# APRIL-ZJU/Ctrl-VIO

Hardware: NVIDIA H100
Metric: residual+Jacobian block evaluations per second (sliding-window LM solve) (higher is better)
Workload: dtype f64

## Files before the change

### ctrl-vio_b200/csrc/chol_dag.cu

```cuda
#include <algorithm>
#include <atomic>
#include <cstdlib>

#include "chol_tiles.cuh"
#include "dmma_tiles.cuh"
#include "kernels.h"

namespace ctvio {

namespace {

__device__ __forceinline__ int ld_acquire(const int* p) {
  int v;
  asm volatile("ld.acquire.gpu.global.s32 %0, [%1];" : "=r"(v) : "l"(p) : "memory");
  return v;
}
__device__ __forceinline__ void st_release(int* p, int v) {
  asm volatile("st.release.gpu.global.s32 [%0], %1;" ::"l"(p), "r"(v) : "memory");
}
constexpr unsigned long long kSentinel = 0xFFF8C0DEC0DE0001ull;
__device__ __forceinline__ unsigned smem_u32(const void* p) { return static_cast<unsigned>(__cvta_generic_to_shared(p)); }
__device__ __forceinline__ unsigned mapa_u32(unsigned addr, unsigned rank) {
  unsigned r;
  asm volatile("mapa.shared::cluster.u32 %0, %1, %2;" : "=r"(r) : "r"(addr), "r"(rank));
  return r;
}
__device__ __forceinline__ void st_cluster2(unsigned addr, double2 v) {
  asm volatile("st.shared::cluster.v2.f64 [%0], {%1, %2};" ::"r"(addr), "d"(v.x), "d"(v.y) : "memory");
}
__device__ __forceinline__ double2 ld_shared_volatile2(const double* p) {
  double2 v;
  asm volatile("ld.volatile.shared.v2.f64 {%0, %1}, [%2];" : "=d"(v.x), "=d"(v.y) : "r"(smem_u32(p)) : "memory");
  return v;
}
__device__ __forceinline__ void cluster_arrive() { asm volatile("barrier.cluster.arrive.release.aligned;" ::: "memory"); }
__device__ __forceinline__ void cluster_wait() { asm volatile("barrier.cluster.wait.acquire.aligned;" ::: "memory"); }
__device__ __forceinline__ unsigned cluster_ctarank() {
  unsigned r;
  asm volatile("mov.u32 %0, %%cluster_ctarank;" : "=r"(r));
  return r;
}
__device__ __forceinline__ unsigned cluster_nctarank() {
// ... 8 lines not shown
  return v;
}
__device__ __forceinline__ void st_relaxed2(double* p, double2 v) {
  asm volatile("st.relaxed.gpu.global.v2.f64 [%0], {%1, %2};" ::"l"(p), "d"(v.x), "d"(v.y) : "memory");
}

__device__ __forceinline__ double ld_relaxed1(const double* p) {
  double v;
  asm volatile("ld.relaxed.gpu.global.f64 %0, [%1];" : "=d"(v) : "l"(p) : "memory");
  return v;
}
__device__ __forceinline__ void st_relaxed1(double* p, double v) {
  asm volatile("st.relaxed.gpu.global.f64 [%0], %1;" ::"l"(p), "d"(v) : "memory");
}
__device__ __forceinline__ double ld_spin(const double* p) {
  double v = ld_relaxed1(p);
  while (is_sentinel(v)) v = ld_relaxed1(p);
  return v;
}
__device__ __forceinline__ double sentinel_value() { return __longlong_as_double(static_cast<long long>(kSentinel)); }

__device__ __forceinline__ void wait_flag(const int* flag, int epoch) {
  if (threadIdx.x == 0) {
    while (ld_acquire(flag) != epoch) {}
  }
  __syncthreads();
}
__device__ __forceinline__ void wait_flags2(const int* f1, const int* f2, int epoch) {
  if (threadIdx.x == 0) {
    while (ld_acquire(f1) != epoch) {}
  } else if (threadIdx.x == 32) {
    while (ld_acquire(f2) != epoch) {}
  }
  __syncthreads();
}
__device__ __forceinline__ void post_flag(int* flag, int epoch) {
  __syncthreads();
  if (threadIdx.x == 0) {
    __threadfence();
    st_release(flag, epoch);
  }
}

__device__ __forceinline__ void load_tile_cg(double* dst, const double* src, int ld, int tid) {
#pragma unroll
  for (int e = tid; e < kCholNB * kCholNB / 2; e += 256) {
    const int r = e >> 5, c = (e & 31) * 2;
    *reinterpret_cast<double2*>(dst + r * kTS + c) = __ldcg(reinterpret_cast<const double2*>(src + size_t(r) * ld + c));
  }
}
__device__ __forceinline__ void store_tile_global(double* dst, int ld, const double* src, int tid) {
#pragma unroll
  for (int e = tid; e < kCholNB * kCholNB / 2; e += 256) {
    const int r = e >> 5, c = (e & 31) * 2;
    *reinterpret_cast<double2*>(dst + size_t(r) * ld + c) = *reinterpret_cast<const double2*>(src + r * kTS + c);
  }
}
__device__ __forceinline__ double sum_partials(const double* part, int n, size_t stride, double* red, int tid) {
  const int c = tid & 63, g = tid >> 6;
  double s = 0.0;
  int q = g;
  for (; q + 12 < n; q += 16) {
    double v0 = ld_relaxed1(part + size_t(q) * stride + c), v1 = ld_relaxed1(part + size_t(q + 4) * stride + c);
// ... 609 lines not shown
```

### ctrl-vio_b200/csrc/engine.cu

```cuda
#include <atomic>
#include <cmath>
#include <cstdlib>
#include <map>

#include "engine_state.h"

namespace ctvio::host {

int refresh_mirror(ctvio_engine* e) {
  const size_t need = 4 * size_t(e->nK) + kPStride * size_t(e->nK) + 6 * size_t(std::max(e->nB, 1)) + size_t(std::max(e->nL, 1)) + 8;
  if (need > e->h_mirror_cap) {
    if (e->h_mirror) cudaFreeHost(e->h_mirror);
    e->h_mirror = nullptr;
    e->h_mirror_cap = 0;
    if (cudaHostAlloc(reinterpret_cast<void**>(&e->h_mirror), (2 * need) * sizeof(double), cudaHostAllocDefault) != cudaSuccess) {
      cudaGetLastError();
      e->mirror_valid = false;
      return CTVIO_OK;
    }
    e->h_mirror_cap = 2 * need;
  }
  DevState& x = e->x[e->cur];
  double* m = e->h_mirror;
  cudaStream_t st = e->stream;
// ... 258 lines not shown
        for (int x = 0; x < nbk; ++x)
          for (int y = 0; y <= x; ++y) {
            lists[size_t(blocks[x]) * (blocks[x] + 1) / 2 + blocks[y]].push_back(l);
            ++total;
          }
      }
      const int n_sm = device_sm_count();
      const int part = std::max(32, int((total / size_t(2 * n_sm) + 31) / 32) * 32);
      std::vector<SchurTileItem> items;
      std::vector<SchurEntry> flat;
      flat.reserve(total);
      for (int ti = 0; ti < T; ++ti)
        for (int tj = 0; tj <= ti; ++tj) {
          const std::vector<int32_t>& v = lists[size_t(ti) * (ti + 1) / 2 + tj];
          for (size_t s0 = 0; s0 < v.size(); s0 += part)
            items.push_back(SchurTileItem{ti, tj, int32_t(flat.size() + s0), int32_t(std::min(v.size() - s0, size_t(part)))});
          for (int32_t l : v) flat.push_back(SchurEntry{l, e->h_lo[l], e->h_hi[l], 0, e->h_woff[l]});
        }
      e->n_schur_items = int(items.size());
      e->n_schur_entries = int(flat.size());
      CUDA_OK(e->d_schur_list.upload(flat, st));
      CUDA_OK(e->d_schur_items.upload(items, st));
    }
    CUDA_OK(e->d_lis.reserve(e->nL));
    CUDA_OK(e->d_lc.reserve(e->nL));
    if (chol_dag_flags_len(e->npad) > e->d_chol_flags.cap) {
      CUDA_OK(e->d_chol_flags.reserve(chol_dag_flags_len(e->npad)));
      CUDA_OK(cudaMemsetAsync(e->d_chol_flags.p, 0, e->d_chol_flags.cap * sizeof(int32_t), e->stream));
    }
    CUDA_OK(e->d_y.reserve(e->npad));
    CUDA_OK(e->d_sc.reserve(np));
    CUDA_OK(e->d_sl.reserve(e->nL));
    CUDA_OK(e->d_hh.reserve(e->nL));
    CUDA_OK(e->d_dc.reserve(np));
    CUDA_OK(e->d_dl.reserve(e->nL));
    if (e->nL > 0) CUDA_OK(cudaMemsetAsync(e->d_hh.p, 0, sizeof(double) * e->nL, st));
    e->prior_dirty = true;
  }
  if (e->structure_dirty || e->masks_dirty) {
    e->h_cmask.assign(d.np, 0);
    for (int k = 0; k < e->nK; ++k)
      if (e->opt.lock_traj || (e->opt.fixed_knot_index >= 0 && k <= e->opt.fixed_knot_index))
        for (int c = 0; c < 6; ++c) e->h_cmask[6 * k + c] = 1;
    for (int b = 0; b < e->nB; ++b)
      for (int c = 0; c < 3; ++c) {
        if (e->opt.lock_wb) e->h_cmask[d.idx_bias0 + 6 * b + c] = 1;
        if (e->opt.lock_ab) e->h_cmask[d.idx_bias0 + 6 * b + 3 + c] = 1;
      }
// ... 146 lines not shown
  v.det_ticket = e->deterministic ? e->d_ticket.p : nullptr;
  return v;
}
SmallFactorsLaunch small_launch(ctvio_engine* e, int xb, int nb) {
  SmallFactorsLaunch v;
  v.bf = BiasFactorPtrs{e->d_bf_ij.p, e->d_bf_s.p, int32_t(e->biasf.size())};
  v.prior = prior_ptrs(e);
  v.st = e->state(xb).ptrs();
  v.ne = e->ne(nb);
  v.dims = e->dims();
  v.cmask = e->d_cmask.p;
  v.scal = e->d_scal.p;
  v.deterministic = e->deterministic ? 1 : 0;
  return v;
}
LinearLaunch linear_launch(ctvio_engine* e, int nb) {
  LinearLaunch a;
  a.dims = e->dims();
  a.ne = e->ne(nb);
  a.lm = e->lml();
  a.schur_list = e->d_schur_list.p;
  a.schur_items = e->d_schur_items.p;
  a.n_schur_items = e->n_schur_items;
  a.lis = e->d_lis.p; a.lc = e->d_lc.p;
  a.cmask = e->d_cmask.p;
  a.active = e->d_active.p;
  a.sc = e->d_sc.p; a.sl = e->d_sl.p;
  a.M = e->d_M.p; a.Linv = e->d_Linv.p; a.y = e->d_y.p;
  a.rhs = e->d_M.p + size_t(e->npad) * e->npad;
  a.diagA = a.rhs + e->npad;
  a.yf = a.diagA + e->npad;
  a.chol_part = e->d_chol_part.p; a.chol_flags = e->d_chol_flags.p; a.chol_seq = &e->chol_seq;
  a.sharded = e->world > 1 ? 1 : 0;
  a.hh = e->d_hh.p; a.dc = e->d_dc.p; a.dl = e->d_dl.p;
  a.npad = e->npad;
  a.scal = e->d_scal.p;
  a.go = nullptr;
  a.det_ticket = e->deterministic ? e->d_ticket.p : nullptr;
  return a;
}

void evaluate(ctvio_engine* e, int xb, int nb, bool full, bool reset_cost) {
  cudaStream_t st = e->stream;
  if (full) {
    if (e->slab_zeroed[nb]) {
      cudaStreamWaitEvent(st, e->ev_zero, 0);
      e->slab_zeroed[nb] = false;
// ... 687 lines not shown
  for (int r = 0; r < reps; ++r) {
    if (r > 0) CUDA_OK(cudaMemcpyAsync(lin.M, backup.p, len * sizeof(double), cudaMemcpyDeviceToDevice, st));
    launch_factor_solve(lin, st);
    CUDA_OK(cudaMemcpyAsync((r == 0 ? x0 : x).data(), lin.y, n * sizeof(double), cudaMemcpyDeviceToHost, st));
    CUDA_OK(cudaStreamSynchronize(st));
    if (r > 0 && std::memcmp(x.data(), x0.data(), n * sizeof(double)) != 0) ++*mismatches;
  }
  for (size_t i = 0; i < n; ++i)
    for (size_t j = i + 1; j < n; ++j) hM[i * n + j] = hM[j * n + i];
  const double* rhs = hM.data() + n * n;
  double rmax = 0, bmax = 0;
  for (size_t i = 0; i < n; ++i) {
    double s = -rhs[i];
    for (size_t j = 0; j < n; ++j) s += hM[i * n + j] * x0[j];
    rmax = std::max(rmax, std::fabs(s));
    bmax = std::max(bmax, std::fabs(rhs[i]));
  }
  *rel_residual = bmax > 0 ? rmax / bmax : rmax;
  cudaMemsetAsync(&e->d_scal.p->error_flags, 0, sizeof(int32_t), st);
  CUDA_OK(cudaStreamSynchronize(st));
  return CTVIO_OK;
}

int ctvio_debug_lm_step(ctvio_handle e, double radius, double* out, int64_t* len) {
  if (!e || !len || !(radius > 0.0)) return fail(CTVIO_ERR_INVALID, "bad argument");
  cudaSetDevice(e->cfg.device);
  int rc = prepare(e);
  if (rc) return rc;
  const ProblemDims d = e->dims();
  const size_t np = size_t(d.np), nL = size_t(e->nL), npad = size_t(e->npad);
  const size_t need = 16 + np * np + np + 2 * nL + nL * np + 2 * np + 2 * nL + npad * npad + 2 * npad + np + nL;
  const int64_t cap = *len;
  *len = int64_t(need);
  if (!out) return CTVIO_OK;
  if (cap < int64_t(need)) return fail(CTVIO_ERR_INVALID, "output slab too small");
  ensure_table(e);
  cudaStream_t st = e->stream;
  const int cur = e->cur;
  evaluate(e, cur, cur, true);
  rc = read_scalars(e);
  if (rc) return rc;
  LinearLaunch lin = linear_launch(e, cur);
  launch_jacobi_scale(lin, st);
  reset_tickets(e);
  launch_reduced_system(lin, radius, st);
  double* o = out + 16;
  double* A = o; o += np * np;
  double* gc = o; o += np;
  double* hl = o; o += nL;
  double* gl = o; o += nL;
  double* W = o; o += nL * np;
  double* cm = o; o += np;
  double* sc = o; o += np;
  double* sl = o; o += nL;
  double* hh = o; o += nL;
  double* M = o; o += npad * npad;
  double* rhs = o; o += npad;
  double* y = o; o += npad;
  double* dc = o; o += np;
  double* dl = o;
  CUDA_OK(cudaMemcpyAsync(M, lin.M, npad * npad * sizeof(double), cudaMemcpyDeviceToHost, st));
  CUDA_OK(cudaMemcpyAsync(rhs, lin.rhs, npad * sizeof(double), cudaMemcpyDeviceToHost, st));
  CUDA_OK(cudaStreamSynchronize(st));
  launch_factor_solve(lin, st);
  CUDA_OK(cudaMemcpyAsync(y, lin.y, npad * sizeof(double), cudaMemcpyDeviceToHost, st));
  CUDA_OK(cudaStreamSynchronize(st));
  launch_step_vectors(lin, st);
// ... 14 lines not shown
    if (!Wc.empty()) CUDA_OK(cudaMemcpyAsync(Wc.data(), ne.W, Wc.size() * sizeof(double), cudaMemcpyDeviceToHost, st));
    CUDA_OK(cudaMemcpyAsync(sl, lin.sl, nL * sizeof(double), cudaMemcpyDeviceToHost, st));
    CUDA_OK(cudaMemcpyAsync(hh, lin.hh, nL * sizeof(double), cudaMemcpyDeviceToHost, st));
    CUDA_OK(cudaMemcpyAsync(dl, lin.dl, nL * sizeof(double), cudaMemcpyDeviceToHost, st));
    CUDA_OK(cudaMemcpyAsync(lo.data(), e->d_lo.p, nL * sizeof(int32_t), cudaMemcpyDeviceToHost, st));
    CUDA_OK(cudaMemcpyAsync(hi.data(), e->d_hi.p, nL * sizeof(int32_t), cudaMemcpyDeviceToHost, st));
    CUDA_OK(cudaMemcpyAsync(woff.data(), e->d_woff.p, nL * sizeof(int64_t), cudaMemcpyDeviceToHost, st));
  }
  CUDA_OK(cudaMemcpyAsync(e->h_scal, e->d_scal.p, sizeof(LmScalars), cudaMemcpyDeviceToHost, st));
  cudaMemsetAsync(&e->d_scal.p->error_flags, 0, sizeof(int32_t), st);
  CUDA_OK(cudaStreamSynchronize(st));
  std::memset(W, 0, nL * np * sizeof(double));
  for (size_t l = 0; l < nL; ++l) {
    for (int g = lo[l]; g < hi[l]; ++g) W[l * np + g] = Wc[size_t(woff[l]) + (g - lo[l])];
    W[l * np + size_t(d.idx_ld)] = wld[l];
  }
  for (size_t i = 0; i < np; ++i) cm[i] = hm[i] ? 1.0 : 0.0;
  const LmScalars& s = *e->h_scal;
  std::memset(out, 0, 16 * sizeof(double));
  out[0] = double(np); out[1] = double(npad); out[2] = double(nL); out[3] = double(e->n_schur_items);
  out[4] = s.gd; out[5] = s.dHd; out[6] = s.dir_max; out[7] = double(s.chol_fail);
  return CTVIO_OK;
}

int ctvio_measure_fp64_tflops(ctvio_handle e, double* tflops) {
  if (!e || !tflops) return fail(CTVIO_ERR_INVALID, "null argument");
  cudaSetDevice(e->cfg.device);
  const double v = ctvio::measure_fp64_tflops(e->stream);
  if (v < 0) return fail(CTVIO_ERR_CUDA, "fp64 micro-benchmark failed");
  *tflops = v;
  return CTVIO_OK;
}

int ctvio_measure_fp64_tensor_tflops(ctvio_handle e, double* tflops) {
  if (!e || !tflops) return fail(CTVIO_ERR_INVALID, "null argument");
  cudaSetDevice(e->cfg.device);
  const double v = ctvio::measure_fp64_tensor_tflops(e->stream);
  if (v < 0) return fail(CTVIO_ERR_CUDA, "fp64 tensor-core micro-benchmark failed");
  *tflops = v;
  return CTVIO_OK;
}

int ctvio_marginalize(ctvio_handle e, int32_t* n_out, int32_t* nb_out) {
  if (!e || !n_out || !nb_out) return fail(CTVIO_ERR_INVALID, "null argument");
  *n_out = 0;
  *nb_out = 0;
// ... 306 lines not shown
```

### ctrl-vio_b200/csrc/engine_state.h

```cpp
#pragma once
#include <algorithm>
#include <cstring>
#include <string>
#include <vector>

#include "../../include/ctvio.h"
#include "frontend.h"
#include "marginalize.h"

namespace ctvio::host {

inline thread_local std::string g_err;
inline int fail(int code, const std::string& msg) {
  g_err = msg;
  return code;
}

#define CUDA_OK(call)                                                                                   \
  do {                                                                                                  \
    cudaError_t e_ = (call);                                                                            \
    if (e_ != cudaSuccess)                                                                              \
      return fail(CTVIO_ERR_CUDA, std::string(#call) + ": " + cudaGetErrorString(e_));                  \
  } while (0)

// ... 114 lines not shown
  DevBuf<int4> d_img_meta;
  DevBuf<int32_t> d_img_orig;
  DevBuf<VisualItem> d_items;
  int n_items = 0;
  std::vector<int32_t> img_order;
  std::vector<int32_t> img_li, img_lj;
  std::vector<int32_t> img_wi0, img_wj0;
  std::vector<VisualItem> h_items;
  std::vector<int32_t> imu_order;
  DevBuf<longlong2> d_imu_t;
  DevBuf<double2> d_imu_ga;
  DevBuf<ImuItem> d_imu_items;
  DevBuf<int32_t> d_imu_orig;
  int n_imu_items = 0;
  DevBuf<int2> d_bf_ij;
  DevBuf<double> d_bf_s;

  std::vector<int32_t> h_lo, h_hi;
  std::vector<int64_t> h_woff;
  DevBuf<int32_t> d_lo, d_hi;
  DevBuf<SchurEntry> d_schur_list;
  DevBuf<int64_t> d_woff;
  DevBuf<SchurTileItem> d_schur_items;
  DevBuf<double> d_lis, d_lc;
  int n_schur_items = 0, n_schur_entries = 0;
  int64_t w_len = 0;
  DevBuf<uint8_t> d_cmask, d_active;
  std::vector<uint8_t> h_cmask, h_active;
  DevBuf<uint64_t> sb_key;
  DevBuf<int32_t> sb_idx;
  DevBuf<uint32_t> sb_counts;
  std::vector<uint32_t> h_struct_counts, img_knots;

  DevBuf<double> ne_slab[2];
  size_t ne_slab_len = 0;
  size_t off_gc = 0, off_hl = 0, off_gl = 0, off_wld = 0, off_W = 0;
  DevBuf<double> d_M, d_Linv, d_y, d_sc, d_sl, d_hh, d_dc, d_dl, d_rho_sync, d_chol_part;
  DevBuf<int32_t> d_chol_flags;
  DevBuf<uint8_t> d_owned;
  DevBuf<double> d_shard_pack, d_shard_scal;
  int npad = 0, linv_npad = -1;
  unsigned chol_seq = 0;
  DevBuf<LmScalars> d_scal;
  LmScalars* h_scal = nullptr;
  LmPublished* h_pub = nullptr;
  unsigned long long pub_seq = 0;
  cudaEvent_t ev_zero = nullptr;
  bool slab_zeroed[2] = {false, false};

  ctvio::PriorHost prior, new_prior;
  DevBuf<double> d_prior_J, d_prior_r, d_prior_JtJ, d_prior_x0, d_prior_dx, d_prior_res;
  DevBuf<int32_t> d_prior_type, d_prior_index, d_prior_col, d_prior_col2g;
  bool prior_dirty = true;
  bool prior_enabled = true;
  bool prior_on_device = false;
  bool new_prior_on_host = false;
  DevBuf<double> d_newprior_x0;
  static constexpr int kFrameSlots = ctvio::kKeyframeMaxSlots, kFrameCap = ctvio::kKeyframeMaxFeatures;
  DevBuf<ctvio::FrameFeature> d_frames;
  DevBuf<int64_t> d_frame_t;
  DevBuf<float> d_cloud_stage;
// ... 102 lines not shown
```

### ctrl-vio_b200/csrc/kernels.h

```cpp
#pragma once
#include <cuda_runtime.h>

#include <atomic>

#include <cstdint>
#include <utility>

#include "spline_eval.cuh"

namespace ctvio {

constexpr int kPStride = 4;
constexpr int kVisThreads = 256;
constexpr int kVisObsPerRound = 128;
constexpr int kVisMinChunk = 64;
constexpr int kLocalDim = 64;
constexpr int kRowStride = 66;
constexpr int kObsStride = 2 * kRowStride + 2;
constexpr int kWinKnots = 5;
constexpr int kColLd = 60, kColR = 61, kColRho = 62;
constexpr int kCholNB = 64;

struct StatePtrs {
  double* q;
// ... 117 lines not shown

struct PerDeviceOnce {
  std::atomic<unsigned long long> mask{0};
  bool first() {
    int d = 0;
    cudaGetDevice(&d);
    const unsigned long long bit = 1ull << (d & 63);
    return !(mask.fetch_or(bit) & bit);
  }
};
inline int device_sm_count() {
  static std::atomic<int> cache[64];
  int d = 0;
  cudaGetDevice(&d);
  int v = cache[d & 63].load(std::memory_order_relaxed);
  if (v == 0) {
    cudaDeviceGetAttribute(&v, cudaDevAttrMultiProcessorCount, d);
    cache[d & 63].store(v, std::memory_order_relaxed);
  }
  return v;
}

#if defined(__CUDACC__)
__device__ __forceinline__ void det_ticket_wait(const int* ticket, int my) {
  if (!ticket) return;
  if (threadIdx.x == 0) {
    int v;
    do { asm volatile("ld.acquire.gpu.global.s32 %0, [%1];" : "=r"(v) : "l"(ticket) : "memory"); } while (v != my);
  }
  __syncthreads();
}
__device__ __forceinline__ void det_ticket_done(int* ticket, int my) {
  if (!ticket) return;
  __threadfence();
  __syncthreads();
  if (threadIdx.x == 0) asm volatile("st.release.gpu.global.s32 [%0], %1;" ::"l"(ticket), "r"(my + 1) : "memory");
}
__device__ __forceinline__ void pdl_wait() { asm volatile("griddepcontrol.wait;" ::: "memory"); }
__device__ __forceinline__ void pdl_launch_dependents() { asm volatile("griddepcontrol.launch_dependents;" ::: "memory"); }
#endif

#if defined(__CUDACC__)
template <typename... KArgs, typename... Args>
cudaError_t launch_chained(bool pdl, void (*kernel)(KArgs...), dim3 grid, dim3 block, size_t smem, cudaStream_t s,
                           Args&&... args) {
  cudaLaunchConfig_t cfg = {};
  cfg.gridDim = grid;
  cfg.blockDim = block;
  cfg.dynamicSmemBytes = smem;
  cfg.stream = s;
  cudaLaunchAttribute at[1];
  at[0].id = cudaLaunchAttributeProgrammaticStreamSerialization;
  at[0].val.programmaticStreamSerializationAllowed = 1;
  cfg.attrs = at;
  cfg.numAttrs = pdl ? 1 : 0;
  return cudaLaunchKernelEx(&cfg, kernel, std::forward<Args>(args)...);
}
#endif

// ... 36 lines not shown
  BiasFactorPtrs bf;
  PriorPtrs prior;
  StatePtrs st;
  NormalEqPtrs ne;
  ProblemDims dims;
  const uint8_t* cmask;
  LmScalars* scal;
  int deterministic = 0;
};
int launch_small_factors(const SmallFactorsLaunch& a, bool full, cudaStream_t s);

int launch_probe_image(const VisualLaunch& a, const int32_t* orig_index, bool want_jac, double* r, int32_t* s,
                       double* J, cudaStream_t st);
int launch_probe_imu(const ImuLaunch& a, const int32_t* orig_index, bool want_jac, double* r, int32_t* s, double* J,
                     cudaStream_t st);

struct LinearLaunch {
  ProblemDims dims;
  NormalEqPtrs ne;
  LandmarkLayout lm;
  const SchurEntry* schur_list;
  const SchurTileItem* schur_items;
  int32_t n_schur_items;
  double* lis;
  double* lc;
  const uint8_t* cmask;
  const uint8_t* active;
  double* sc;
  double* sl;
  double* M;
  double* Linv;
  double* rhs;
  double* y;
  double* yf;
  double* chol_part;
  int32_t* chol_flags;
  unsigned* chol_seq;
  double* hh;
  double* diagA;
  int32_t sharded;
  double* dc;
  double* dl;
  int32_t npad;
  LmScalars* scal;
  int* det_ticket;
  const int32_t* go;
  int32_t pdl = 0;
};
int launch_jacobi_scale(const LinearLaunch& a, cudaStream_t s);
int launch_lm_step(const LinearLaunch& a, double radius, cudaStream_t s);
int launch_reduced_system(const LinearLaunch& a, double radius, cudaStream_t s, const double* radius_dev = nullptr);
int launch_factor_solve(const LinearLaunch& a, cudaStream_t s);
bool chol_dag_supported(int npad, int n_sm);
size_t chol_dag_part_len(int npad);
size_t chol_dag_flags_len(int npad);
size_t chol_dag_lpub_len(int npad);
int launch_chol_dag_init(double* linv_buf, double* part_buf, int npad, cudaStream_t s);
int launch_chol_dag(const LinearLaunch& a, cudaStream_t s);
int launch_chol_coop(const LinearLaunch& a, cudaStream_t s);
int launch_step_vectors(const LinearLaunch& a, cudaStream_t s);
int launch_extract_diag(const LinearLaunch& a, cudaStream_t s);
int launch_jacobi_scale_from_diag(const LinearLaunch& a, cudaStream_t s);
int launch_gradient_norm(const LinearLaunch& a, const StatePtrs& st, int fix_ld, double ld_lower, double ld_upper,
                         cudaStream_t s, bool reset = true, LmPublished* pub = nullptr, unsigned long long seq = 0,
                         const LmDecideArgs* decide = nullptr);

struct ApplyLaunch {
  int32_t count_camera;
  ProblemDims dims;
  StatePtrs x, xc;
  const double* dc;
  const double* dl;
  double alpha;
  const uint8_t* active;
// ... 21 lines not shown
```

### ctrl-vio_b200/csrc/kernels_linear.cu

```cuda
#include <algorithm>

#include "dmma_tiles.cuh"
#include <cstddef>

#include "kernels.h"

namespace ctvio {

__device__ __forceinline__ double warp_sum_d(double v) {
#pragma unroll
  for (int o = 16; o > 0; o >>= 1) v += __shfl_xor_sync(0xffffffffu, v, o);
  return v;
}
__device__ __forceinline__ double warp_max_d(double v) {
#pragma unroll
  for (int o = 16; o > 0; o >>= 1) v = fmax(v, __shfl_xor_sync(0xffffffffu, v, o));
  return v;
}
__device__ __forceinline__ void atomic_max_pos(double* addr, double v) {
  atomicMax(reinterpret_cast<unsigned long long*>(addr), static_cast<unsigned long long>(__double_as_longlong(v)));
}

constexpr double kMinLmDiag = 1e-6, kMaxLmDiag = 1e32;

__global__ void jacobi_scale_kernel(LinearLaunch a) {
  const int i = blockIdx.x * blockDim.x + threadIdx.x;
  const int np = a.dims.np;
  if (i < np) a.sc[i] = 1.0 / (1.0 + sqrt(a.ne.A[size_t(i) * np + i]));
  if (i < a.dims.nL) a.sl[i] = 1.0 / (1.0 + sqrt(a.ne.hl[i]));
}
int launch_jacobi_scale(const LinearLaunch& a, cudaStream_t s) {
  const int n = max(a.dims.np, a.dims.nL);
  jacobi_scale_kernel<<<(n + 255) / 256, 256, 0, s>>>(a);
  return 1;
}

__global__ void scale_copy_kernel(LinearLaunch a, double radius, const double* __restrict__ radius_dev) {
  pdl_wait();
  pdl_launch_dependents();
  if (radius_dev) radius = *radius_dev;
  const int npad = a.npad, np = a.dims.np;
  const size_t idx = size_t(blockIdx.x) * blockDim.x + threadIdx.x;
  if (idx < size_t(a.dims.nL)) {
    const int l = int(idx);
    const double sl = a.sl[l], hl = a.ne.hl[l];
    const double hs = sl * sl * hl;
    const double hh = hl > 0.0 ? hs + fmin(fmax(hs, kMinLmDiag), kMaxLmDiag) / radius : 0.0;
    const double is = hh > 0.0 ? rsqrt(hh) * sl : 0.0;
    a.hh[l] = hh;
    a.lis[l] = is;
    a.lc[l] = is * a.ne.gl[l];
  }
  if (idx >= size_t(npad) * npad) return;
  const int i = int(idx / npad), j = int(idx % npad);
  double m;
  const double ident = a.sharded ? 0.0 : 1.0;
  if (i < np && j < np) {
    if (a.cmask[i] || a.cmask[j]) {
      m = (i == j) ? ident : 0.0;
    } else {
      const double v = (i <= j) ? a.ne.A[size_t(i) * np + j] : a.ne.A[size_t(j) * np + i];
      m = a.sc[i] * v * a.sc[j];
      if (i == j) {
        if (a.sharded) a.diagA[i] = v;
        else m += fmin(fmax(m, kMinLmDiag), kMaxLmDiag) / radius;
      }
    }
  } else {
    m = (i == j) ? ident : 0.0;
    if (a.sharded && i == j) a.diagA[i] = 0.0;
  }
  if (a.sharded && i == j && i < np && a.cmask[i]) a.diagA[i] = 0.0;
  a.M[idx] = m;
  if (j == 0) {
    a.rhs[i] = (i < np && !a.cmask[i]) ? a.sc[i] * a.ne.gc[i] : 0.0;
    if (i == 0) {
      a.scal->gd = 0.0;
      a.scal->dHd = 0.0;
      a.scal->dir_max = 0.0;
      a.scal->chol_fail = 0;
      a.scal->step_norm2 = 0.0;
      a.scal->x_norm2 = 0.0;
      a.scal->cost_eval = 0.0;
      a.scal->gmax = 0.0;
    }
  }
}

constexpr int kSchurKC = 32;
__device__ __forceinline__ void schur_fetch(const LinearLaunch& a, const SchurTileItem& it, int c0, int k, int dseg,
                                            const double* scA, const double* scB, double sc_ld, bool diag, double va[8],
                                            double vb[8], double cl[3]) {
#pragma unroll
  for (int e = 0; e < 8; ++e) va[e] = vb[e] = 0.0;
  cl[0] = cl[1] = cl[2] = 0.0;
  if (c0 + k >= it.count) return;
  const SchurEntry en = a.schur_list[it.first + c0 + k];
  const double is = a.lis[en.l];
  const double* Wl = a.ne.W + en.woff - en.lo;
  const int ga0 = kCholNB * it.ti + dseg, gb0 = kCholNB * it.tj + dseg;
  cl[0] = a.lc[en.l];
  cl[1] = is * a.ne.wld[en.l] * sc_ld;
  cl[2] = en.lo / kCholNB == it.ti ? 1.0 : 0.0;
  if (ga0 + 8 > en.lo && ga0 < en.hi) {
#pragma unroll
    for (int e = 0; e < 8; ++e)
      if (ga0 + e >= en.lo && ga0 + e < en.hi) va[e] = is * Wl[ga0 + e] * scA[dseg + e];
  }
  if (!diag && gb0 + 8 > en.lo && gb0 < en.hi) {
#pragma unroll
    for (int e = 0; e < 8; ++e)
      if (gb0 + e >= en.lo && gb0 + e < en.hi) vb[e] = is * Wl[gb0 + e] * scB[dseg + e];
  }
}

__global__ void __launch_bounds__(256, 2) schur_tile_kernel(LinearLaunch a) {
  __shared__ __align__(16) double At[kSchurKC * kTS];
  __shared__ __align__(16) double Bt[kSchurKC * kTS];
  __shared__ double scA[kCholNB], scB[kCholNB], cvec[3][kSchurKC];
  const SchurTileItem it = a.schur_items[blockIdx.x];
  const int tid = threadIdx.x;
  const Lane L = lane_of(tid);
  const int np = a.dims.np, npad = a.npad, ild = a.dims.idx_ld;
  const bool diag = it.ti == it.tj;
  if (tid < kCholNB) {
    const int ga = kCholNB * it.ti + tid, gb = kCholNB * it.tj + tid;
    scA[tid] = (ga < np && !a.cmask[ga]) ? a.sc[ga] : 0.0;
    scB[tid] = (gb < np && !a.cmask[gb]) ? a.sc[gb] : 0.0;
  }
  const double sc_ld = a.cmask[ild] ? 0.0 : a.sc[ild];
  const int go = a.go ? *a.go : 1;
  __syncthreads();
  pdl_wait();
  pdl_launch_dependents();
  if (!go) return;
  Frag acc;
  frag_zero(acc);
  double racc = 0.0, lacc = 0.0, ll = 0.0, lr = 0.0;
  const int k = tid >> 3, dseg = (tid & 7) * 8;
  double va[8], vb[8], cl[3];
  schur_fetch(a, it, 0, k, dseg, scA, scB, sc_ld, diag, va, vb, cl);
  for (int c0 = 0; c0 < it.count; c0 += kSchurKC) {
#pragma unroll
    for (int e = 0; e < 8; e += 2) {
      *reinterpret_cast<double2*>(At + k * kTS + dseg + e) = make_double2(va[e], va[e + 1]);
      if (!diag) *reinterpret_cast<double2*>(Bt + k * kTS + dseg + e) = make_double2(vb[e], vb[e + 1]);
    }
    if ((tid & 7) == 0) { cvec[0][k] = cl[0]; cvec[1][k] = cl[1]; cvec[2][k] = cl[2]; }
    __syncthreads();
    if (c0 + kSchurKC < it.count) schur_fetch(a, it, c0 + kSchurKC, k, dseg, scA, scB, sc_ld, diag, va, vb, cl);
    tile_gemm_dmma<false, kSchurKC>(At, diag ? At : Bt, acc, L);
    if (diag) {
      if (tid < kCholNB) {
#pragma unroll 8
        for (int kk = 0; kk < kSchurKC; ++kk) {
          const double v = At[kk * kTS + tid];
          racc = fma(v, cvec[0][kk], racc);
          lacc = fma(v, cvec[1][kk], lacc);
        }
      } else if (tid < kCholNB + kSchurKC) {
        const int kk = tid - kCholNB;
        const double vld = cvec[1][kk] * cvec[2][kk];
        ll = fma(vld, cvec[1][kk], ll);
        lr = fma(vld, cvec[0][kk], lr);
      }
    }
    __syncthreads();
  }
  det_ticket_wait(a.det_ticket, blockIdx.x);
  double* tile = a.M + size_t(kCholNB) * it.ti * npad + kCholNB * it.tj;
#pragma unroll
  for (int mt = 0; mt < 2; ++mt)
#pragma unroll
    for (int nt = 0; nt < 4; ++nt)
#pragma unroll
      for (int e = 0; e < 2; ++e) {
        const double v = acc.c[mt][nt][e];
        if (v != 0.0) atomicAdd(tile + size_t(L.row(mt)) * npad + L.col(nt) + e, -v);
      }
  if (diag) {
    if (tid < kCholNB) {
      if (racc != 0.0) atomicAdd(a.rhs + kCholNB * it.ti + tid, -racc);
      if (lacc != 0.0) atomicAdd(a.M + size_t(ild) * npad + kCholNB * it.ti + tid, -lacc);
    } else if (tid < kCholNB + kSchurKC) {
      ll = warp_sum_d(ll);
      lr = warp_sum_d(lr);
      if (tid == kCholNB) {
        if (ll != 0.0) atomicAdd(a.M + size_t(ild) * npad + ild, -ll);
        if (lr != 0.0) atomicAdd(a.rhs + ild, -lr);
      }
    }
  }
  det_ticket_done(a.det_ticket, blockIdx.x);
}


__device__ __forceinline__ void camera_step_block(const LinearLaunch& a, int block, double* dsh) {
  __shared__ double red[3][8];
  const int np = a.dims.np;
  const int i = block * 8 + (threadIdx.x >> 5);
  const int lane = threadIdx.x & 31;
  double gd = 0, dHd = 0, dmax = 0;
  const int j0 = block * 8;
  for (int j = j0 + threadIdx.x; j < np; j += blockDim.x) dsh[j - j0] = a.cmask[j] ? 0.0 : -a.sc[j] * a.y[j];
  __syncthreads();
  if (i < np) {
    const double di = dsh[i - j0];
    if (lane == 0) {
      a.dc[i] = di;
      gd = a.ne.gc[i] * di;
      dmax = fabs(di);
      if (!isfinite(di)) a.scal->chol_fail = 1;
    }
    if (di != 0.0) {
      double s = 0;
      for (int j = i + lane; j < np; j += 32) s = fma(a.ne.A[size_t(i) * np + j] * (j == i ? 0.5 : 1.0), dsh[j - j0], s);
// ... 67 lines not shown
}

__global__ void extract_diag_kernel(LinearLaunch a) {
  const int i = blockIdx.x * blockDim.x + threadIdx.x;
  if (i >= a.npad) return;
  a.diagA[i] = i < a.dims.np ? a.ne.A[size_t(i) * a.dims.np + i] : 0.0;
}
int launch_extract_diag(const LinearLaunch& a, cudaStream_t s) {
  extract_diag_kernel<<<(a.npad + 255) / 256, 256, 0, s>>>(a);
  return 1;
}
__global__ void jacobi_scale_from_diag_kernel(LinearLaunch a) {
  const int i = blockIdx.x * blockDim.x + threadIdx.x;
  if (i < a.dims.np) a.sc[i] = 1.0 / (1.0 + sqrt(a.diagA[i]));
  if (i < a.dims.nL) a.sl[i] = 1.0 / (1.0 + sqrt(a.ne.hl[i]));
}
int launch_jacobi_scale_from_diag(const LinearLaunch& a, cudaStream_t s) {
  const int n = max(a.dims.np, a.dims.nL);
  jacobi_scale_from_diag_kernel<<<(n + 255) / 256, 256, 0, s>>>(a);
  return 1;
}

int launch_reduced_system(const LinearLaunch& a, double radius, cudaStream_t s, const double* radius_dev) {
  int launches = 0;
  const size_t total = std::max(size_t(a.npad) * a.npad, size_t(a.dims.nL));
  launch_chained(a.pdl, scale_copy_kernel, dim3(unsigned((total + 255) / 256)), dim3(256), 0, s, a, radius, radius_dev);
  ++launches;
  if (a.n_schur_items > 0) {
    launch_chained(a.pdl, schur_tile_kernel, dim3(a.n_schur_items), dim3(256), 0, s, a);
    ++launches;
  }
  return launches;
}

int launch_step_vectors(const LinearLaunch& a, cudaStream_t s) {
  const int ncb = (a.dims.np + 7) / 8, nlb = (a.dims.nL + 7) / 8;
  step_vectors_kernel<<<ncb + nlb, 256, size_t(a.dims.np) * sizeof(double), s>>>(a, ncb);
  return 1;
}

int launch_lm_step(const LinearLaunch& a, double radius, cudaStream_t s) {
  return launch_reduced_system(a, radius, s) + launch_factor_solve(a, s) + launch_step_vectors(a, s);
}

__global__ void __launch_bounds__(1024) gradient_norm_kernel(LinearLaunch a, StatePtrs st, int fix_ld, double ld_lower,
                                                             double ld_upper, LmPublished* pub, unsigned long long seq,
                                                             LmDecideArgs da) {
  __shared__ double red[32];
  pdl_wait();
  pdl_launch_dependents();
  const int np = a.dims.np, nL = a.dims.nL;
  double v = 0.0;
  for (int i = blockIdx.x * blockDim.x + threadIdx.x; i < np + nL; i += gridDim.x * blockDim.x) {
    if (!a.active[i]) continue;
    double x;
// ... 234 lines not shown
```

Before: 35.49 million.

## Fuse scale-copy and Schur tile kernels into one flag-synchronized reduced-system kernel

Merges the scale/copy pass that builds the scaled reduced matrix and the Schur-complement tile kernel into a single launch. Base-tile blocks write their tile of M and release a per-tile epoch flag, and Schur item blocks spin on those flags before atomically subtracting their contributions. The landmark inverse-sqrt and gradient scalars are now recomputed inside the Schur blocks instead of being staged in global lis/lc buffers, which removes a launch boundary and two global arrays. The risk is spin-wait deadlock if item blocks occupy the device before the base blocks are scheduled. Base blocks also change the copy of A to a shared-memory transpose, which costs some redundant per-row arithmetic.

Result: faster. 37.58 million, median of 6 (+5.9%).

```diff
diff --git a/ctrl-vio_b200/csrc/chol_dag.cu b/ctrl-vio_b200/csrc/chol_dag.cu
--- a/ctrl-vio_b200/csrc/chol_dag.cu
+++ b/ctrl-vio_b200/csrc/chol_dag.cu
@@ -10,14 +10,6 @@
 
 namespace {
 
-__device__ __forceinline__ int ld_acquire(const int* p) {
-  int v;
-  asm volatile("ld.acquire.gpu.global.s32 %0, [%1];" : "=r"(v) : "l"(p) : "memory");
-  return v;
-}
-__device__ __forceinline__ void st_release(int* p, int v) {
-  asm volatile("st.release.gpu.global.s32 [%0], %1;" ::"l"(p), "r"(v) : "memory");
-}
 constexpr unsigned long long kSentinel = 0xFFF8C0DEC0DE0001ull;
 __device__ __forceinline__ unsigned smem_u32(const void* p) { return static_cast<unsigned>(__cvta_generic_to_shared(p)); }
 __device__ __forceinline__ unsigned mapa_u32(unsigned addr, unsigned rank) {
@@ -72,15 +64,15 @@
 
 __device__ __forceinline__ void wait_flag(const int* flag, int epoch) {
   if (threadIdx.x == 0) {
-    while (ld_acquire(flag) != epoch) {}
+    spin_until_gpu(flag, epoch);
   }
   __syncthreads();
 }
 __device__ __forceinline__ void wait_flags2(const int* f1, const int* f2, int epoch) {
   if (threadIdx.x == 0) {
-    while (ld_acquire(f1) != epoch) {}
+    spin_until_gpu(f1, epoch);
   } else if (threadIdx.x == 32) {
-    while (ld_acquire(f2) != epoch) {}
+    spin_until_gpu(f2, epoch);
   }
   __syncthreads();
 }
@@ -88,7 +80,7 @@
   __syncthreads();
   if (threadIdx.x == 0) {
     __threadfence();
-    st_release(flag, epoch);
+    st_release_gpu(flag, epoch);
   }
 }
 
diff --git a/ctrl-vio_b200/csrc/engine.cu b/ctrl-vio_b200/csrc/engine.cu
--- a/ctrl-vio_b200/csrc/engine.cu
+++ b/ctrl-vio_b200/csrc/engine.cu
@@ -304,8 +304,10 @@
       CUDA_OK(e->d_schur_list.upload(flat, st));
       CUDA_OK(e->d_schur_items.upload(items, st));
     }
-    CUDA_OK(e->d_lis.reserve(e->nL));
-    CUDA_OK(e->d_lc.reserve(e->nL));
+    if (reduced_system_flags_len(e->npad) > e->d_m_flags.cap) {
+      CUDA_OK(e->d_m_flags.reserve(reduced_system_flags_len(e->npad)));
+      CUDA_OK(cudaMemsetAsync(e->d_m_flags.p, 0, e->d_m_flags.cap * sizeof(int32_t), e->stream));
+    }
     if (chol_dag_flags_len(e->npad) > e->d_chol_flags.cap) {
       CUDA_OK(e->d_chol_flags.reserve(chol_dag_flags_len(e->npad)));
       CUDA_OK(cudaMemsetAsync(e->d_chol_flags.p, 0, e->d_chol_flags.cap * sizeof(int32_t), e->stream));
@@ -498,7 +500,7 @@
   a.schur_list = e->d_schur_list.p;
   a.schur_items = e->d_schur_items.p;
   a.n_schur_items = e->n_schur_items;
-  a.lis = e->d_lis.p; a.lc = e->d_lc.p;
+  a.m_flags = e->d_m_flags.p;
   a.cmask = e->d_cmask.p;
   a.active = e->d_active.p;
   a.sc = e->d_sc.p; a.sl = e->d_sl.p;
@@ -1232,7 +1234,7 @@
   return CTVIO_OK;
 }
 
-int ctvio_debug_lm_step(ctvio_handle e, double radius, double* out, int64_t* len) {
+int ctvio_debug_lm_step_poison(ctvio_handle e, double radius, double* out, int64_t* len, int32_t poison) {
   if (!e || !len || !(radius > 0.0)) return fail(CTVIO_ERR_INVALID, "bad argument");
   cudaSetDevice(e->cfg.device);
   int rc = prepare(e);
@@ -1253,6 +1255,7 @@
   LinearLaunch lin = linear_launch(e, cur);
   launch_jacobi_scale(lin, st);
   reset_tickets(e);
+  if (poison) CUDA_OK(cudaMemsetAsync(lin.M, 0xff, (npad * npad + npad) * sizeof(double), st));
   launch_reduced_system(lin, radius, st);
   double* o = out + 16;
   double* A = o; o += np * np;
@@ -1313,6 +1316,9 @@
   out[4] = s.gd; out[5] = s.dHd; out[6] = s.dir_max; out[7] = double(s.chol_fail);
   return CTVIO_OK;
 }
+int ctvio_debug_lm_step(ctvio_handle e, double radius, double* out, int64_t* len) {
+  return ctvio_debug_lm_step_poison(e, radius, out, len, 0);
+}
 
 int ctvio_measure_fp64_tflops(ctvio_handle e, double* tflops) {
   if (!e || !tflops) return fail(CTVIO_ERR_INVALID, "null argument");
diff --git a/ctrl-vio_b200/csrc/engine_state.h b/ctrl-vio_b200/csrc/engine_state.h
--- a/ctrl-vio_b200/csrc/engine_state.h
+++ b/ctrl-vio_b200/csrc/engine_state.h
@@ -160,7 +160,6 @@
   DevBuf<SchurEntry> d_schur_list;
   DevBuf<int64_t> d_woff;
   DevBuf<SchurTileItem> d_schur_items;
-  DevBuf<double> d_lis, d_lc;
   int n_schur_items = 0, n_schur_entries = 0;
   int64_t w_len = 0;
   DevBuf<uint8_t> d_cmask, d_active;
@@ -174,7 +173,7 @@
   size_t ne_slab_len = 0;
   size_t off_gc = 0, off_hl = 0, off_gl = 0, off_wld = 0, off_W = 0;
   DevBuf<double> d_M, d_Linv, d_y, d_sc, d_sl, d_hh, d_dc, d_dl, d_rho_sync, d_chol_part;
-  DevBuf<int32_t> d_chol_flags;
+  DevBuf<int32_t> d_chol_flags, d_m_flags;
   DevBuf<uint8_t> d_owned;
   DevBuf<double> d_shard_pack, d_shard_scal;
   int npad = 0, linv_npad = -1;
diff --git a/ctrl-vio_b200/csrc/kernels.h b/ctrl-vio_b200/csrc/kernels.h
--- a/ctrl-vio_b200/csrc/kernels.h
+++ b/ctrl-vio_b200/csrc/kernels.h
@@ -163,19 +163,27 @@
 }
 
 #if defined(__CUDACC__)
+__device__ __forceinline__ int ld_acquire_gpu(const int* p) {
+  int v;
+  asm volatile("ld.acquire.gpu.global.s32 %0, [%1];" : "=r"(v) : "l"(p) : "memory");
+  return v;
+}
+__device__ __forceinline__ void st_release_gpu(int* p, int v) {
+  asm volatile("st.release.gpu.global.s32 [%0], %1;" ::"l"(p), "r"(v) : "memory");
+}
+__device__ __forceinline__ void spin_until_gpu(const int* p, int v) {
+  while (ld_acquire_gpu(p) != v) {}
+}
 __device__ __forceinline__ void det_ticket_wait(const int* ticket, int my) {
   if (!ticket) return;
-  if (threadIdx.x == 0) {
-    int v;
-    do { asm volatile("ld.acquire.gpu.global.s32 %0, [%1];" : "=r"(v) : "l"(ticket) : "memory"); } while (v != my);
-  }
+  if (threadIdx.x == 0) spin_until_gpu(ticket, my);
   __syncthreads();
 }
 __device__ __forceinline__ void det_ticket_done(int* ticket, int my) {
   if (!ticket) return;
   __threadfence();
   __syncthreads();
-  if (threadIdx.x == 0) asm volatile("st.release.gpu.global.s32 [%0], %1;" ::"l"(ticket), "r"(my + 1) : "memory");
+  if (threadIdx.x == 0) st_release_gpu(ticket, my + 1);
 }
 __device__ __forceinline__ void pdl_wait() { asm volatile("griddepcontrol.wait;" ::: "memory"); }
 __device__ __forceinline__ void pdl_launch_dependents() { asm volatile("griddepcontrol.launch_dependents;" ::: "memory"); }
@@ -258,8 +266,7 @@
   const SchurEntry* schur_list;
   const SchurTileItem* schur_items;
   int32_t n_schur_items;
-  double* lis;
-  double* lc;
+  int32_t* m_flags;
   const uint8_t* cmask;
   const uint8_t* active;
   double* sc;
@@ -286,6 +293,7 @@
 int launch_jacobi_scale(const LinearLaunch& a, cudaStream_t s);
 int launch_lm_step(const LinearLaunch& a, double radius, cudaStream_t s);
 int launch_reduced_system(const LinearLaunch& a, double radius, cudaStream_t s, const double* radius_dev = nullptr);
+size_t reduced_system_flags_len(int npad);
 int launch_factor_solve(const LinearLaunch& a, cudaStream_t s);
 bool chol_dag_supported(int npad, int n_sm);
 size_t chol_dag_part_len(int npad);
diff --git a/ctrl-vio_b200/csrc/kernels_linear.cu b/ctrl-vio_b200/csrc/kernels_linear.cu
--- a/ctrl-vio_b200/csrc/kernels_linear.cu
+++ b/ctrl-vio_b200/csrc/kernels_linear.cu
@@ -1,4 +1,5 @@
 #include <algorithm>
+#include <atomic>
 
 #include "dmma_tiles.cuh"
 #include <cstddef>
@@ -35,90 +36,150 @@
   return 1;
 }
 
-__global__ void scale_copy_kernel(LinearLaunch a, double radius, const double* __restrict__ radius_dev) {
+constexpr int kSchurKC = 32;
+constexpr int kBaseTS = kCholNB + 1;
+static_assert(kCholNB * kBaseTS <= 2 * kSchurKC * kTS, "the base tile lives in the item operands' shared memory");
+
+__host__ __device__ __forceinline__ int lower_tile_index(int ti, int tj) { return ti * (ti + 1) / 2 + tj; }
+size_t reduced_system_flags_len(int npad) {
+  const int T = npad / kCholNB;
+  return size_t(lower_tile_index(T, 0));
+}
+
+__device__ __forceinline__ double landmark_hh(double sl, double hl, double radius) {
+  const double hs = sl * sl * hl;
+  return hl > 0.0 ? hs + fmin(fmax(hs, kMinLmDiag), kMaxLmDiag) / radius : 0.0;
+}
+__device__ __forceinline__ double landmark_is(double hh, double sl) { return hh > 0.0 ? rsqrt(hh) * sl : 0.0; }
+
+__device__ __forceinline__ void reduced_base_block(const LinearLaunch& a, int b, double radius, const double* radius_dev,
+                                                   int epoch, double* Ts, double* scR, double* scC, uint8_t* cmR,
+                                                   uint8_t* cmC) {
+  const int tid = threadIdx.x;
+  int ti = 0;
+  while (lower_tile_index(ti + 1, 0) <= b) ++ti;
+  const int tj = b - lower_tile_index(ti, 0);
+  const int npad = a.npad, np = a.dims.np;
+  const int r0 = kCholNB * ti, c0 = kCholNB * tj;
+#pragma unroll
+  for (int k = 0; k < kCholNB * kCholNB / 256; ++k) {
+    const int e = tid + 256 * k, x = e / kCholNB, y = e % kCholNB;
+    Ts[x * kBaseTS + y] = (c0 + x < np && r0 + y < np) ? a.ne.A[size_t(c0 + x) * np + r0 + y] : 0.0;
+  }
+  const int nbase = lower_tile_index(npad / kCholNB, 0), l0 = b * 256 + tid;
+  const double sl0 = l0 < a.dims.nL ? a.sl[l0] : 0.0, hl0 = l0 < a.dims.nL ? a.ne.hl[l0] : 0.0;
+  double rg = 0.0;
+  if (tid < kCholNB) {
+    const int i = r0 + tid, j = c0 + tid;
+    scR[tid] = i < np ? a.sc[i] : 0.0;
+    cmR[tid] = i < np ? a.cmask[i] : 1;
+    scC[tid] = j < np ? a.sc[j] : 0.0;
+    cmC[tid] = j < np ? a.cmask[j] : 1;
+    if (ti == tj && i < np) rg = a.ne.gc[i];
+  }
+  __syncthreads();
   pdl_wait();
   pdl_launch_dependents();
   if (radius_dev) radius = *radius_dev;
-  const int npad = a.npad, np = a.dims.np;
-  const size_t idx = size_t(blockIdx.x) * blockDim.x + threadIdx.x;
-  if (idx < size_t(a.dims.nL)) {
-    const int l = int(idx);
-    const double sl = a.sl[l], hl = a.ne.hl[l];
-    const double hs = sl * sl * hl;
-    const double hh = hl > 0.0 ? hs + fmin(fmax(hs, kMinLmDiag), kMaxLmDiag) / radius : 0.0;
-    const double is = hh > 0.0 ? rsqrt(hh) * sl : 0.0;
-    a.hh[l] = hh;
-    a.lis[l] = is;
-    a.lc[l] = is * a.ne.gl[l];
-  }
-  if (idx >= size_t(npad) * npad) return;
-  const int i = int(idx / npad), j = int(idx % npad);
-  double m;
   const double ident = a.sharded ? 0.0 : 1.0;
-  if (i < np && j < np) {
-    if (a.cmask[i] || a.cmask[j]) {
+  double* tile = a.M + size_t(r0) * npad + c0;
+#pragma unroll 4
+  for (int k = 0; k < kCholNB * kCholNB / 256; ++k) {
+    const int e = tid + 256 * k, rr = e / kCholNB, cc = e % kCholNB;
+    const int i = r0 + rr, j = c0 + cc;
+    double m;
+    if (i < np && j < np) {
+      if (cmR[rr] || cmC[cc]) {
+        m = (i == j) ? ident : 0.0;
+      } else {
+        const double v = (i <= j) ? Ts[rr * kBaseTS + cc] : Ts[cc * kBaseTS + rr];
+        m = scR[rr] * v * scC[cc];
+        if (i == j) {
+          if (a.sharded) a.diagA[i] = v;
+          else m += fmin(fmax(m, kMinLmDiag), kMaxLmDiag) / radius;
+        }
+      }
+    } else {
       m = (i == j) ? ident : 0.0;
-    } else {
-      const double v = (i <= j) ? a.ne.A[size_t(i) * np + j] : a.ne.A[size_t(j) * np + i];
-      m = a.sc[i] * v * a.sc[j];
-      if (i == j) {
-        if (a.sharded) a.diagA[i] = v;
-        else m += fmin(fmax(m, kMinLmDiag), kMaxLmDiag) / radius;
-      }
-    }
-  } else {
-    m = (i == j) ? ident : 0.0;
-    if (a.sharded && i == j) a.diagA[i] = 0.0;
-  }
-  if (a.sharded && i == j && i < np && a.cmask[i]) a.diagA[i] = 0.0;
-  a.M[idx] = m;
-  if (j == 0) {
-    a.rhs[i] = (i < np && !a.cmask[i]) ? a.sc[i] * a.ne.gc[i] : 0.0;
-    if (i == 0) {
-      a.scal->gd = 0.0;
-      a.scal->dHd = 0.0;
-      a.scal->dir_max = 0.0;
-      a.scal->chol_fail = 0;
-      a.scal->step_norm2 = 0.0;
-      a.scal->x_norm2 = 0.0;
-      a.scal->cost_eval = 0.0;
-      a.scal->gmax = 0.0;
-    }
-  }
-}
-
-constexpr int kSchurKC = 32;
-__device__ __forceinline__ void schur_fetch(const LinearLaunch& a, const SchurTileItem& it, int c0, int k, int dseg,
-                                            const double* scA, const double* scB, double sc_ld, bool diag, double va[8],
-                                            double vb[8], double cl[3]) {
-#pragma unroll
-  for (int e = 0; e < 8; ++e) va[e] = vb[e] = 0.0;
-  cl[0] = cl[1] = cl[2] = 0.0;
+      if (a.sharded && i == j) a.diagA[i] = 0.0;
+    }
+    if (a.sharded && i == j && i < np && cmR[rr]) a.diagA[i] = 0.0;
+    tile[size_t(rr) * npad + cc] = m;
+  }
+  if (ti == tj && tid < kCholNB) a.rhs[r0 + tid] = (r0 + tid < np && !cmR[tid]) ? scR[tid] * rg : 0.0;
+  __syncthreads();
+  if (tid == 0) {
+    __threadfence();
+    st_release_gpu(a.m_flags + b, epoch);
+  }
+  if (l0 < a.dims.nL) a.hh[l0] = landmark_hh(sl0, hl0, radius);
+  for (int l = l0 + nbase * 256; l < a.dims.nL; l += nbase * 256) a.hh[l] = landmark_hh(a.sl[l], a.ne.hl[l], radius);
+  if (b == 0 && tid == 0) {
+    a.scal->gd = 0.0;
+    a.scal->dHd = 0.0;
+    a.scal->dir_max = 0.0;
+    a.scal->chol_fail = 0;
+    a.scal->step_norm2 = 0.0;
+    a.scal->x_norm2 = 0.0;
+    a.scal->cost_eval = 0.0;
+    a.scal->gmax = 0.0;
+  }
+}
+
+struct SchurRow {
+  double va[8], vb[8];
+  double sl, hl, gl, wld;
+  int32_t lo, hi;
+};
+__device__ __forceinline__ void schur_load(const LinearLaunch& a, const SchurTileItem& it, int c0, int k, int dseg, bool diag,
+                                           SchurRow& r) {
+#pragma unroll
+  for (int e = 0; e < 8; ++e) r.va[e] = r.vb[e] = 0.0;
+  r.lo = -1;
   if (c0 + k >= it.count) return;
   const SchurEntry en = a.schur_list[it.first + c0 + k];
-  const double is = a.lis[en.l];
   const double* Wl = a.ne.W + en.woff - en.lo;
   const int ga0 = kCholNB * it.ti + dseg, gb0 = kCholNB * it.tj + dseg;
-  cl[0] = a.lc[en.l];
-  cl[1] = is * a.ne.wld[en.l] * sc_ld;
-  cl[2] = en.lo / kCholNB == it.ti ? 1.0 : 0.0;
+  r.lo = en.lo;
+  r.hi = en.hi;
+  r.sl = a.sl[en.l];
+  r.hl = a.ne.hl[en.l];
+  r.gl = a.ne.gl[en.l];
+  r.wld = a.ne.wld[en.l];
   if (ga0 + 8 > en.lo && ga0 < en.hi) {
 #pragma unroll
     for (int e = 0; e < 8; ++e)
-      if (ga0 + e >= en.lo && ga0 + e < en.hi) va[e] = is * Wl[ga0 + e] * scA[dseg + e];
+      if (ga0 + e >= en.lo && ga0 + e < en.hi) r.va[e] = Wl[ga0 + e];
   }
   if (!diag && gb0 + 8 > en.lo && gb0 < en.hi) {
 #pragma unroll
     for (int e = 0; e < 8; ++e)
-      if (gb0 + e >= en.lo && gb0 + e < en.hi) vb[e] = is * Wl[gb0 + e] * scB[dseg + e];
-  }
-}
-
-__global__ void __launch_bounds__(256, 2) schur_tile_kernel(LinearLaunch a) {
-  __shared__ __align__(16) double At[kSchurKC * kTS];
-  __shared__ __align__(16) double Bt[kSchurKC * kTS];
-  __shared__ double scA[kCholNB], scB[kCholNB], cvec[3][kSchurKC];
-  const SchurTileItem it = a.schur_items[blockIdx.x];
+      if (gb0 + e >= en.lo && gb0 + e < en.hi) r.vb[e] = Wl[gb0 + e];
+  }
+}
+__device__ __forceinline__ void schur_scale(const SchurTileItem& it, int dseg, const double* scA, const double* scB,
+                                            double sc_ld, bool diag, double radius, SchurRow& r, double cl[3]) {
+  cl[0] = cl[1] = cl[2] = 0.0;
+  if (r.lo < 0) return;
+  const double is = landmark_is(landmark_hh(r.sl, r.hl, radius), r.sl);
+  const int ga0 = kCholNB * it.ti + dseg, gb0 = kCholNB * it.tj + dseg;
+  cl[0] = is * r.gl;
+  cl[1] = is * r.wld * sc_ld;
+  cl[2] = r.lo / kCholNB == it.ti ? 1.0 : 0.0;
+#pragma unroll
+  for (int e = 0; e < 8; ++e)
+    if (ga0 + e >= r.lo && ga0 + e < r.hi) r.va[e] = is * r.va[e] * scA[dseg + e];
+  if (!diag) {
+#pragma unroll
+    for (int e = 0; e < 8; ++e)
+      if (gb0 + e >= r.lo && gb0 + e < r.hi) r.vb[e] = is * r.vb[e] * scB[dseg + e];
+  }
+}
+
+__device__ __forceinline__ void reduced_item_block(const LinearLaunch& a, int item, double radius, const double* radius_dev,
+                                                   int epoch, double* At, double* Bt, double* scA, double* scB,
+                                                   double (*cvec)[kSchurKC]) {
+  const SchurTileItem it = a.schur_items[item];
   const int tid = threadIdx.x;
   const Lane L = lane_of(tid);
   const int np = a.dims.np, npad = a.npad, ild = a.dims.idx_ld;
@@ -129,26 +190,29 @@
     scB[tid] = (gb < np && !a.cmask[gb]) ? a.sc[gb] : 0.0;
   }
   const double sc_ld = a.cmask[ild] ? 0.0 : a.sc[ild];
-  const int go = a.go ? *a.go : 1;
+  const int k = tid >> 3, dseg = (tid & 7) * 8;
+  SchurRow row;
+  schur_load(a, it, 0, k, dseg, diag, row);
   __syncthreads();
   pdl_wait();
   pdl_launch_dependents();
+  const int go = a.go ? *a.go : 1;
+  if (radius_dev) radius = *radius_dev;
   if (!go) return;
   Frag acc;
   frag_zero(acc);
   double racc = 0.0, lacc = 0.0, ll = 0.0, lr = 0.0;
-  const int k = tid >> 3, dseg = (tid & 7) * 8;
-  double va[8], vb[8], cl[3];
-  schur_fetch(a, it, 0, k, dseg, scA, scB, sc_ld, diag, va, vb, cl);
   for (int c0 = 0; c0 < it.count; c0 += kSchurKC) {
+    double cl[3];
+    schur_scale(it, dseg, scA, scB, sc_ld, diag, radius, row, cl);
 #pragma unroll
     for (int e = 0; e < 8; e += 2) {
-      *reinterpret_cast<double2*>(At + k * kTS + dseg + e) = make_double2(va[e], va[e + 1]);
-      if (!diag) *reinterpret_cast<double2*>(Bt + k * kTS + dseg + e) = make_double2(vb[e], vb[e + 1]);
+      *reinterpret_cast<double2*>(At + k * kTS + dseg + e) = make_double2(row.va[e], row.va[e + 1]);
+      if (!diag) *reinterpret_cast<double2*>(Bt + k * kTS + dseg + e) = make_double2(row.vb[e], row.vb[e + 1]);
     }
     if ((tid & 7) == 0) { cvec[0][k] = cl[0]; cvec[1][k] = cl[1]; cvec[2][k] = cl[2]; }
     __syncthreads();
-    if (c0 + kSchurKC < it.count) schur_fetch(a, it, c0 + kSchurKC, k, dseg, scA, scB, sc_ld, diag, va, vb, cl);
+    if (c0 + kSchurKC < it.count) schur_load(a, it, c0 + kSchurKC, k, dseg, diag, row);
     tile_gemm_dmma<false, kSchurKC>(At, diag ? At : Bt, acc, L);
     if (diag) {
       if (tid < kCholNB) {
@@ -167,7 +231,14 @@
     }
     __syncthreads();
   }
-  det_ticket_wait(a.det_ticket, blockIdx.x);
+  {
+    const int tl = ild / kCholNB;
+    if (tid == 0) spin_until_gpu(a.m_flags + lower_tile_index(it.ti, it.tj), epoch);
+    else if (diag && tid == 32) spin_until_gpu(a.m_flags + lower_tile_index(tl, it.ti), epoch);
+    else if (diag && tid == 64) spin_until_gpu(a.m_flags + lower_tile_index(tl, tl), epoch);
+    __syncthreads();
+  }
+  det_ticket_wait(a.det_ticket, item);
   double* tile = a.M + size_t(kCholNB) * it.ti * npad + kCholNB * it.tj;
 #pragma unroll
   for (int mt = 0; mt < 2; ++mt)
@@ -191,7 +262,17 @@
       }
     }
   }
-  det_ticket_done(a.det_ticket, blockIdx.x);
+  det_ticket_done(a.det_ticket, item);
+}
+
+__global__ void __launch_bounds__(256, 2) reduced_system_kernel(LinearLaunch a, double radius,
+                                                                const double* __restrict__ radius_dev, int epoch) {
+  __shared__ __align__(16) double opnd[2 * kSchurKC * kTS];
+  __shared__ double scA[kCholNB], scB[kCholNB], cvec[3][kSchurKC];
+  __shared__ uint8_t cmA[kCholNB], cmB[kCholNB];
+  const int nbase = lower_tile_index(a.npad / kCholNB, 0);
+  if (int(blockIdx.x) < nbase) reduced_base_block(a, blockIdx.x, radius, radius_dev, epoch, opnd, scA, scB, cmA, cmB);
+  else reduced_item_block(a, blockIdx.x - nbase, radius, radius_dev, epoch, opnd, opnd + kSchurKC * kTS, scA, scB, cvec);
 }
 
 
@@ -305,15 +386,12 @@
 }
 
 int launch_reduced_system(const LinearLaunch& a, double radius, cudaStream_t s, const double* radius_dev) {
-  int launches = 0;
-  const size_t total = std::max(size_t(a.npad) * a.npad, size_t(a.dims.nL));
-  launch_chained(a.pdl, scale_copy_kernel, dim3(unsigned((total + 255) / 256)), dim3(256), 0, s, a, radius, radius_dev);
-  ++launches;
-  if (a.n_schur_items > 0) {
-    launch_chained(a.pdl, schur_tile_kernel, dim3(a.n_schur_items), dim3(256), 0, s, a);
-    ++launches;
-  }
-  return launches;
+  static std::atomic<unsigned> epoch_src{0};
+  const int epoch = int(epoch_src.fetch_add(1, std::memory_order_relaxed) % 0x7ffffffeu) + 1;
+  const int nbase = lower_tile_index(a.npad / kCholNB, 0);
+  launch_chained(a.pdl, reduced_system_kernel, dim3(unsigned(nbase + a.n_schur_items)), dim3(256), 0, s, a, radius,
+                 radius_dev, epoch);
+  return 1;
 }
 
 int launch_step_vectors(const LinearLaunch& a, cudaStream_t s) {
```
